# Edward-Sun/DIFUSCO

Measured on NVIDIA H100. Metric: TSP-500 graphs/sec, 50-step categorical denoise, higher is better.
Workload: dtype f32 (3-term bf16 split on wgmma, fp32 accumulate)

## Files before the change

### difusco_b200/_cabi.py

```python
import ctypes as C
import os

import numpy as np

HERE = os.path.dirname(os.path.abspath(__file__))
LIB_PATH = os.path.join(HERE, "libdifusco_b200.so")

DFB_OK, DFB_E_INVALID, DFB_E_CUDA, DFB_E_UNSUPPORTED, DFB_E_NOMEM = 0, -1, -2, -3, -4
CATEGORICAL, GAUSSIAN = 0, 1
EDGE_IMPL_TC, EDGE_IMPL_FP32, EDGE_IMPL_TC1 = 0, 1, 2
AGGREGATION = {"sum": 0, "mean": 1, "max": 2}
HEAD_FORWARD, HEAD_CATEGORICAL, HEAD_GAUSSIAN = 0, 1, 2

SYMBOLS = [
    "dfb_abi_version", "dfb_create", "dfb_destroy", "dfb_last_error", "dfb_set_aggregation",
    "dfb_set_edge_impl", "dfb_load_weights", "dfb_prepare_graph", "dfb_prepare_graph_instances", "dfb_set_points",
    "dfb_encoder_forward", "dfb_encoder_forward_timesteps", "dfb_denoise_step", "dfb_denoise", "dfb_denoise_record", "dfb_denoise_instances",
    "dfb_denoise_host",
    "dfb_launch_count", "dfb_profile_begin", "dfb_profile_end", "dfb_debug_edge_gemm", "dfb_debug_gnn_layer",
    "dfb_debug_gnn_layer_timesteps", "dfb_debug_head", "dfb_debug_entry", "dfb_debug_loop_captures",
    "dfb_debug_phase_cycles", "dfb_debug_watchdog", "dfb_knn_graph", "dfb_set_graph_capture",
    "dfb_set_phase_timing", "dfb_tsp_merge_sparse", "dfb_tsp_merge_order", "dfb_two_opt", "dfb_two_opt_instances",
    "dfb_write_heatmap_txt",
]

_lib = None


def lib():
  global _lib
  if _lib is not None:
    return _lib
  if not os.path.exists(LIB_PATH):
    raise RuntimeError(
        f"{LIB_PATH} not found: build it with `python -m difusco_b200.build` "
        "(difusco_b200 has no fallback path; the CUDA library is the product)")
  L = C.CDLL(LIB_PATH)
  vp, i32, i64, u64, f32 = C.c_void_p, C.c_int, C.c_int64, C.c_uint64, C.c_float
  L.dfb_abi_version.restype = i32
  L.dfb_create.argtypes = [C.POINTER(vp), i32]
  L.dfb_destroy.argtypes = [vp]
  L.dfb_last_error.argtypes = [vp]
  L.dfb_last_error.restype = C.c_char_p
  L.dfb_set_aggregation.argtypes = [vp, i32]
  L.dfb_set_edge_impl.argtypes = [vp, i32]
  L.dfb_load_weights.argtypes = [vp, i32, i32, i32, i32, i32, C.POINTER(C.c_char_p), C.POINTER(vp),
                                 C.POINTER(i64)]
  L.dfb_prepare_graph.argtypes = [vp, vp, i64, i64, i32, vp]
  L.dfb_prepare_graph_instances.argtypes = [vp, vp, i64, i64, i32, C.POINTER(i64), vp]
  L.dfb_set_points.argtypes = [vp, vp, vp]
  L.dfb_encoder_forward.argtypes = [vp, vp, f32, vp, vp]
  L.dfb_encoder_forward_timesteps.argtypes = [vp, vp, i32, C.POINTER(f32), vp, vp, vp]
  L.dfb_denoise_step.argtypes = [vp, i32, vp, f32, C.POINTER(f32), i32, vp, u64, i32, vp, vp, vp, vp]
  L.dfb_denoise.argtypes = [vp, i32, vp, i32, C.POINTER(C.c_int32), C.POINTER(f32),
                            C.POINTER(C.c_int32), vp, u64, vp]
  L.dfb_denoise_record.argtypes = [vp, i32, vp, i32, C.POINTER(C.c_int32), C.POINTER(f32), C.POINTER(C.c_int32), vp,
                                   u64, i32, C.POINTER(C.c_int32), vp, vp, vp, vp]
  L.dfb_denoise_instances.argtypes = [vp, i32, vp, i32, C.POINTER(C.c_int32), C.POINTER(f32), C.POINTER(C.c_int32),
                                      vp, i32, i32, C.POINTER(C.c_int32), vp, vp, vp, vp]
  L.dfb_denoise_host.argtypes = [vp, i32, vp, vp, i64, i64, i32, vp, i32, C.POINTER(C.c_int32),
                                 C.POINTER(f32), C.POINTER(C.c_int32), u64, vp, vp]
  L.dfb_launch_count.argtypes = [vp]
  L.dfb_launch_count.restype = i64
  L.dfb_debug_loop_captures.argtypes = [vp]
  L.dfb_debug_loop_captures.restype = i64
  L.dfb_profile_begin.argtypes = [vp]
  L.dfb_profile_end.argtypes = [vp, C.POINTER(C.c_double), C.POINTER(i64)]
  L.dfb_debug_edge_gemm.argtypes = [vp, i32, vp, vp, vp]
  L.dfb_debug_gnn_layer.argtypes = [vp, i32, f32, vp, vp, vp]
  L.dfb_debug_gnn_layer_timesteps.argtypes = [vp, i32, i32, C.POINTER(f32), vp, vp, vp, vp]
  L.dfb_debug_head.argtypes = [vp, i32, vp, C.POINTER(f32), i32, vp, u64, i32, vp, vp, vp, vp, vp, vp, vp]
  L.dfb_debug_entry.argtypes = [vp, i32, vp, f32, vp, vp, vp, vp, vp, vp]
  L.dfb_debug_phase_cycles.argtypes = [vp, C.POINTER(C.c_uint64)]
  L.dfb_debug_watchdog.argtypes = [vp, C.POINTER(C.c_int)]
  L.dfb_set_graph_capture.argtypes = [vp, i32]
  L.dfb_set_phase_timing.argtypes = [vp, i32]
  L.dfb_knn_graph.argtypes = [vp, vp, i64, i32, i64, vp, vp]
  L.dfb_tsp_merge_sparse.argtypes = [vp, i64, vp, vp, i64, i32, vp, C.POINTER(i64)]
  L.dfb_tsp_merge_order.argtypes = [i64, vp, i64, vp, C.POINTER(i64)]
  L.dfb_two_opt.argtypes = [vp, vp, i64, vp, i64, i64, C.POINTER(i64), vp]
  L.dfb_two_opt_instances.argtypes = [vp, vp, vp, i64, vp, vp, i64, vp, vp]
  L.dfb_write_heatmap_txt.argtypes = [C.c_char_p, i64, vp]
  for name in SYMBOLS:
    fn = getattr(L, name)
    if fn.restype is C.c_int and name not in ("dfb_abi_version",):
      fn.restype = i32
  _lib = L
  return L


class DfbError(RuntimeError):
  pass


def _raise(code, msg):
  msg = msg.decode() if isinstance(msg, bytes) else msg
  if code == DFB_E_INVALID:
    raise ValueError(msg)
  if code == DFB_E_UNSUPPORTED:
    raise NotImplementedError(msg)
  if code == DFB_E_NOMEM:
    raise MemoryError(msg)
  raise DfbError(msg)


MERGE_COMPLETE, MERGE_INCOMPLETE, MERGE_AMBIGUOUS = 0, 1, 2

# ... 212 lines not shown
                                         its.ctypes.data, stream))
    out, e = [], 0
    for p, t in zip(points_list, tours_list):
      b, n1 = np.shape(t)
      out.append(tours[e:e + b * n1].reshape(b, n1))
      e += b * n1
    return out, [int(x) for x in its]

  def knn_graph(self, points_ptr, num_nodes, k, node_offset, edge_index_ptr, stream=0):
    self._ck(lib().dfb_knn_graph(self._h, points_ptr, int(num_nodes), int(k), int(node_offset), edge_index_ptr, stream))

  def launch_count(self):
    return int(lib().dfb_launch_count(self._h))

  def loop_captures(self):
    return int(lib().dfb_debug_loop_captures(self._h))

  def profile_begin(self):
    self._ck(lib().dfb_profile_begin(self._h))

  def profile_end(self):
    ms, n = C.c_double(0), C.c_int64(0)
    self._ck(lib().dfb_profile_end(self._h, C.byref(ms), C.byref(n)))
    return ms.value, n.value

  def set_graph_capture(self, enabled):
    self._ck(lib().dfb_set_graph_capture(self._h, int(bool(enabled))))

  def debug_watchdog(self):
    out = (C.c_int * 4)()
    lib().dfb_debug_watchdog(self._h, out)
    return [int(x) for x in out]

  def set_phase_timing(self, enabled):
    self._ck(lib().dfb_set_phase_timing(self._h, int(bool(enabled))))

  def debug_phase_cycles(self):
    out = (C.c_uint64 * 32)()
    self._ck(lib().dfb_debug_phase_cycles(self._h, out))
    return [int(x) for x in out]

  def debug_edge_gemm(self, layer, e_in_ptr, acc_out_ptr, stream=0):
    self._ck(lib().dfb_debug_edge_gemm(self._h, layer, e_in_ptr, acc_out_ptr, stream))

  def debug_gnn_layer(self, layer, t, h_ptr, e_ptr, stream=0):
    self._ck(lib().dfb_debug_gnn_layer(self._h, int(layer), float(t), h_ptr, e_ptr, stream))

  def debug_gnn_layer_timesteps(self, layer, t_values, t_index_ptr, h_ptr, e_ptr, stream=0):
    v = np.ascontiguousarray(t_values, dtype=np.float32).reshape(-1)
    self._ck(lib().dfb_debug_gnn_layer_timesteps(self._h, int(layer), v.size, v.ctypes.data_as(C.POINTER(C.c_float)),
                                                 t_index_ptr, h_ptr, e_ptr, stream))

  def debug_head(self, mode, z_ptr, consts=(0, 0, 0, 0), last=0, uniforms_ptr=None, seed=0, step_index=0,
                 instance_seeds_ptr=None, xt_in_ptr=None, xt_out_ptr=None, p_out_ptr=None, net_out_ptr=None,
                 stats_out_ptr=None, stream=0):
    c = (C.c_float * 4)(*[float(x) for x in consts])
    self._ck(lib().dfb_debug_head(self._h, int(mode), z_ptr, c, int(last), uniforms_ptr,
                                  int(seed) & 0xFFFFFFFFFFFFFFFF, int(step_index), instance_seeds_ptr, xt_in_ptr,
                                  xt_out_ptr, p_out_ptr, net_out_ptr, stats_out_ptr, stream))

  def debug_entry(self, diffusion, xt_ptr, t, h0_out_ptr=None, e0_out_ptr=None, tvec_out_ptr=None, h_out_ptr=None,
                  e_out_ptr=None, stream=0):
    self._ck(lib().dfb_debug_entry(self._h, int(diffusion), xt_ptr, float(t), h0_out_ptr, e0_out_ptr, tvec_out_ptr,
                                   h_out_ptr, e_out_ptr, stream))
```

### difusco_b200/csrc/dfb_api.cu

```cuda
#include <cuda_runtime.h>
#include <math.h>
#include <stdio.h>
#include <stdlib.h>
#include <string.h>

#include <map>
#include <string>
#include <vector>

#include "../../include/difusco_b200.h"
#include "common.cuh"
#include "edge_layer_fp32.cuh"
#include "edge_layer_tc.cuh"
#include "kernels_small.cuh"
#include "knn.cuh"
#include "tsp_decode.cuh"

using namespace dfb;

static std::string g_create_error;

struct DevBuf {
  void* p = nullptr;
  size_t cap = 0;
// ... 1232 lines not shown
  ctx->h_tvals[slot][0] = t;
  ctx->h_steps[slot][0] = StepParams{};
  r = stage_commit(ctx, slot, 1, st);
  if (r) return r;
  const float* xt_lut;
  int e_zero;
  r = run_entry(ctx, mode, xt, &xt_lut, &e_zero, st);
  if (r) return r;
  const size_t V = ctx->g.V, E = ctx->g.E, row = H * sizeof(float);
  if (h0_out) CK(ctx, cudaMemcpyAsync(h0_out, ctx->h.p, V * row, cudaMemcpyDeviceToDevice, st));
  if (e0_out && xt_lut) {
    k_lut_expand<<<(ctx->g.E + 3) / 4, 256, 0, st>>>(xt_lut, ctx->g.perm, ctx->lut, e0_out, ctx->g.E);
    CKL(ctx);
  } else if (e0_out && !e_zero) {
    CK(ctx, cudaMemcpyAsync(e0_out, ctx->e.p, E * row, cudaMemcpyDeviceToDevice, st));
  }
  if (tvec_out) CK(ctx, cudaMemcpyAsync(tvec_out, ctx->tvec.p, ctx->L * row, cudaMemcpyDeviceToDevice, st));
  r = run_forward_layer(ctx, 0, (const float*)ctx->tvec.p, TimeRows{}, xt_lut, e_zero, st);
  if (r) return r;
  if (h_out) CK(ctx, cudaMemcpyAsync(h_out, ctx->h.p, V * row, cudaMemcpyDeviceToDevice, st));
  if (e_out) CK(ctx, cudaMemcpyAsync(e_out, ctx->e.p, E * row, cudaMemcpyDeviceToDevice, st));
  return DFB_OK;
}

extern "C" int dfb_debug_phase_cycles(dfb_ctx* ctx, unsigned long long* out) {
  if (!ctx || !out) return DFB_E_INVALID;
  CK(ctx, cudaSetDevice(ctx->device));
  CK(ctx, cudaDeviceSynchronize());
  CK(ctx, cudaMemcpy(out, ctx->tc.phase_cycles, 32 * sizeof(unsigned long long), cudaMemcpyDeviceToHost));
  CK(ctx, cudaMemset(ctx->tc.phase_cycles, 0, 32 * sizeof(unsigned long long)));
  return DFB_OK;
}

extern "C" int dfb_debug_watchdog(dfb_ctx* ctx, int* out) {
  if (!ctx || !out || !ctx->tc.error_host) return DFB_E_INVALID;
  for (int i = 0; i < 4; ++i) out[i] = ((volatile int*)ctx->tc.error_host)[i];
  return DFB_OK;
}

extern "C" int dfb_knn_graph(dfb_ctx* ctx, const double* points, int64_t num_nodes, int k, int64_t node_offset,
                             int64_t* edge_index, void* stream_) {
  if (!ctx) return DFB_E_INVALID;
  cudaStream_t st = (cudaStream_t)stream_;
  CK(ctx, cudaSetDevice(ctx->device));
  if (num_nodes < 1 || k < 1 || k > num_nodes) FAIL(ctx, DFB_E_INVALID, "bad kNN size N=%lld K=%d", (long long)num_nodes, k);
  if ((size_t)num_nodes * sizeof(double) > 200 * 1024) FAIL(ctx, DFB_E_UNSUPPORTED, "kNN graph: N=%lld exceeds the shared-memory brute-force limit (25600)", (long long)num_nodes);
  const size_t smem = (size_t)num_nodes * sizeof(double) + (size_t)(num_nodes + 31) / 32 * sizeof(unsigned);
  if (!is_device_ptr(edge_index)) FAIL(ctx, DFB_E_INVALID, "edge_index must be a device pointer");
  const double* dp = points;
  if (!is_device_ptr(points)) {
    for (int64_t i = 0; i < 2 * num_nodes; ++i)
      if (!std::isfinite(points[i])) FAIL(ctx, DFB_E_INVALID, "kNN graph: non-finite coordinate of node %lld", (long long)(i / 2));
    ENS_NOLOOP(ctx, ctx->d_points, (size_t)num_nodes * 2 * sizeof(double));
    CK(ctx, cudaMemcpyAsync(ctx->d_points.p, points, (size_t)num_nodes * 2 * sizeof(double), cudaMemcpyHostToDevice, st));
    dp = (const double*)ctx->d_points.p;
  }
  CK(ctx, cudaFuncSetAttribute(k_knn_bruteforce, cudaFuncAttributeMaxDynamicSharedMemorySize, (int)smem));
  k_knn_bruteforce<<<(int)num_nodes, 256, smem, st>>>(dp, (int)num_nodes, k, (long long*)edge_index, (long long)node_offset);
  CKL(ctx);
  return DFB_OK;
}

extern "C" int dfb_tsp_merge_sparse(const double* points, int64_t n, const float* heat, const int64_t* edge_index, int64_t E,
                                    int mode, int64_t* tour, int64_t* merge_iterations) {
  if (!points || !heat || !edge_index || !tour || !merge_iterations || n < 3 || n > 0x7fffffff / 2 || E < 0 || (mode != 0 && mode != 1))
    return DFB_E_INVALID;
// ... 146 lines not shown
```

### difusco_b200/csrc/edge_layer_tc.cuh

```cuda
#pragma once
#include <cuda.h>
#include <cuda_bf16.h>
#include <cuda_runtime.h>

#include <stdlib.h>

#include <string>

#include "common.cuh"
#include "edge_layer_fp32.cuh"

namespace dfb {

constexpr int WG_ROWS = 64;
constexpr int TC_KBLK = 64;
constexpr int TC_KCH = 32;
constexpr int TC_B_BYTES = 256 * TC_KCH * 2;
static_assert(TC_KCH * 2 == 64, "weight chunk rows are one 64-byte swizzle row (tensor map, wgmma_desc_sw64)");
constexpr int TC_A_CHUNK = WG_ROWS * 128;
constexpr int TC_A_BYTES = 8 * TC_A_CHUNK;
constexpr int CONV_BATCH = 16;

constexpr int W_LO_ROWS = H;
constexpr int W_MAT_ROWS = 2 * W_LO_ROWS;
// ... 56 lines not shown
  asm volatile("mbarrier.arrive.shared::cta.b64 _, [%0];" ::"r"(smem_u32(bar)) : "memory");
}
__device__ __forceinline__ void mbar_arrive_expect_tx(uint64_t* bar, uint32_t bytes) {
  asm volatile("mbarrier.arrive.expect_tx.shared::cta.b64 _, [%0], %1;" ::"r"(smem_u32(bar)), "r"(bytes) : "memory");
}
__device__ __forceinline__ void mbar_wait(uint64_t* bar, uint32_t parity, int* error_flag, int code) {
  const uint32_t addr = smem_u32(bar);
  uint32_t ok = 0;
#pragma unroll 1
  for (uint32_t spin = 0;; ++spin) {
    asm volatile(
        "{\n .reg .pred p;\n mbarrier.try_wait.parity.shared::cta.b64 p, [%1], %2, %3;\n selp.u32 %0, 1, 0, p;\n}"
        : "=r"(ok)
        : "r"(addr), "r"(parity), "r"(20000u)
        : "memory");
    if (ok) return;
    if (spin > 400000u) {
      if (error_flag) {
        error_flag[1] = (int)blockIdx.x;
        error_flag[2] = (int)parity;
        error_flag[3] = (int)threadIdx.x;
        atomicExch(error_flag, code);
      }
      __threadfence_system();
      __trap();
    }
  }
}
__device__ __forceinline__ void tma_load_2d(uint32_t dst, const CUtensorMap* map, uint64_t* bar, int c0, int c1) {
  asm volatile(
      "cp.async.bulk.tensor.2d.shared::cluster.global.mbarrier::complete_tx::bytes [%0], [%1, {%3, %4}], [%2];"
      ::"r"(dst), "l"(reinterpret_cast<uint64_t>(map)), "r"(smem_u32(bar)), "r"(c0), "r"(c1)
      : "memory");
}
__device__ __forceinline__ void fence_proxy_async() { asm volatile("fence.proxy.async.shared::cta;" ::: "memory"); }
__device__ __forceinline__ void cp_async16(void* dst, const void* src) {
  asm volatile("cp.async.cg.shared.global [%0], [%1], 16;" ::"r"(smem_u32(dst)), "l"(src) : "memory");
}
__device__ __forceinline__ void cp_async_commit() { asm volatile("cp.async.commit_group;" ::: "memory"); }
__device__ __forceinline__ void cp_async_wait_all() { asm volatile("cp.async.wait_group 0;" ::: "memory"); }

__device__ __forceinline__ uint64_t wgmma_desc_sw128(uint32_t smem_addr) {
  return (uint64_t)((smem_addr >> 4) & 0x3fffu) | (1ull << 16) | (64ull << 32) | (1ull << 62);
}
__device__ __forceinline__ uint64_t wgmma_desc_sw64(uint32_t smem_addr) {
  return (uint64_t)((smem_addr >> 4) & 0x3fffu) | (1ull << 16) | (32ull << 32) | (2ull << 62);
}
__device__ __forceinline__ void wgmma_fence() { asm volatile("wgmma.fence.sync.aligned;" ::: "memory"); }
__device__ __forceinline__ void wgmma_commit() { asm volatile("wgmma.commit_group.sync.aligned;" ::: "memory"); }
template <int N>
__device__ __forceinline__ void wgmma_wait() { asm volatile("wgmma.wait_group.sync.aligned %0;" ::"n"(N) : "memory"); }
__device__ __forceinline__ void acc_fence(float (&d)[128]) {
#pragma unroll
  for (int i = 0; i < 128; ++i) asm volatile("" : "+f"(d[i])::"memory");
}
__device__ __forceinline__ void wgmma_bf16(float (&d)[128], uint64_t da, uint64_t db, uint32_t scale_d) {
  asm volatile(
      "{\n .reg .pred p;\n setp.ne.b32 p, %130, 0;\n"
      "wgmma.mma_async.sync.aligned.m64n256k16.f32.bf16.bf16 "
      "{%0, %1, %2, %3, %4, %5, %6, %7, %8, %9, %10, %11, %12, %13, %14, %15, "
      "%16, %17, %18, %19, %20, %21, %22, %23, %24, %25, %26, %27, %28, %29, %30, %31, "
      "%32, %33, %34, %35, %36, %37, %38, %39, %40, %41, %42, %43, %44, %45, %46, %47, "
      "%48, %49, %50, %51, %52, %53, %54, %55, %56, %57, %58, %59, %60, %61, %62, %63, "
      "%64, %65, %66, %67, %68, %69, %70, %71, %72, %73, %74, %75, %76, %77, %78, %79, "
      "%80, %81, %82, %83, %84, %85, %86, %87, %88, %89, %90, %91, %92, %93, %94, %95, "
      "%96, %97, %98, %99, %100, %101, %102, %103, %104, %105, %106, %107, %108, %109, %110, %111, "
// ... 45 lines not shown
  return (uint32_t)((r >> 3) * 1024 + (r & 7) * 128 + ((j ^ (r & 7)) << 4));
}
__device__ __forceinline__ int msg_col(int j, int r) { return 64 * (j >> 3) + ((8 * (j & 7)) ^ (8 * (r & 7))); }
__device__ __forceinline__ float quad_sum(float v) {
  v += __shfl_xor_sync(0xffffffffu, v, 1);
  return v + __shfl_xor_sync(0xffffffffu, v, 2);
}
__device__ __forceinline__ void swap_row_halves(float (&d)[128]) {
#pragma unroll
  for (int j = 0; j < 32; ++j) {
    const float x0 = d[4 * j], x1 = d[4 * j + 1];
    d[4 * j] = d[4 * j + 2];
    d[4 * j + 1] = d[4 * j + 3];
    d[4 * j + 2] = x0;
    d[4 * j + 3] = x1;
  }
}

enum {
  PH_TILES = 0,
  PH_TOTAL,
  PH_CONVERT,
  PH_G1_WAIT,
  PH_G1_MMA,
  PH_E1,
  PH_REDUCE,
  PH_LN,
  PH_G2_WAIT,
  PH_G2_MMA,
  PH_E4,
  PH_COUNT
};

template <int NWG, bool LIN, bool TIMED = false, bool TROWS = false>
__device__ __forceinline__ void edge_layer_wg_body(const CUtensorMap& wmap, const TcParams& P) {
  using Cfg = TcCfg<NWG>;
  constexpr int NSTAGE = Cfg::NSTAGE;
  extern __shared__ unsigned char smem_raw[];
  unsigned char* smem = smem_raw + ((1024u - (smem_u32(smem_raw) & 1023u)) & 1023u);
  float* prm = reinterpret_cast<float*>(smem + Cfg::OFF_PRM);
  int* s_row = reinterpret_cast<int*>(smem + Cfg::OFF_ROW);
  const float** s_src = reinterpret_cast<const float**>(smem + Cfg::OFF_SRC);
  const float** s_tau = reinterpret_cast<const float**>(smem + Cfg::OFF_TAU);
  uint64_t* full = reinterpret_cast<uint64_t*>(smem + Cfg::OFF_BAR);
  uint64_t* empty = full + NSTAGE;

  const int warp = threadIdx.x >> 5, lane = threadIdx.x & 31;
  constexpr bool lin = LIN;
  const int loads_per_tile = (P.write_e ? 2 : 1) * NWG * 4 * NSTAGE;

  if (threadIdx.x == 0) {
    for (int s = 0; s < NSTAGE; ++s) {
      mbar_init(&full[s], 1);
      mbar_init(&empty[s], 4);
    }
    asm volatile("fence.mbarrier_init.release.cluster;" ::: "memory");
    fence_proxy_async();
  }
  for (int i = threadIdx.x; i < H; i += Cfg::THREADS) {
    prm[i] = P.lp.ln_e_g[i];
    prm[H + i] = P.lp.ln_e_b[i];
    prm[2 * H + i] = P.tvec ? P.tvec[i] : 0.0f;
    prm[3 * H + i] = P.lp.ln_o_g[i];
    prm[4 * H + i] = P.lp.ln_o_b[i];
    prm[5 * H + i] = P.lp.b_O[i];
  }
  __syncthreads();
  const uint32_t smem_base = smem_u32(smem);

  if (warp >= 4 * NWG) {
    if constexpr (NWG == 2) asm volatile("setmaxnreg.dec.sync.aligned.u32 40;" ::: "memory");
    if (warp == 4 * NWG && lane == 0) {
      uint32_t u = 0;
      for (int tile = blockIdx.x; tile < P.n_tiles; tile += gridDim.x) {
        for (int i = 0; i < loads_per_tile; ++i, ++u) {
          const int s = u % NSTAGE;
          mbar_wait(&empty[s], ((u / NSTAGE) & 1) ^ 1, P.error_flag, 1);
          mbar_arrive_expect_tx(&full[s], TC_B_BYTES);
          const int row = (lin ? P.lin_w_row + (P.lin_nb == 4 ? (tile & 3) : 0) * W_MAT_ROWS
                               : P.w_row_base + (i >= 4 * NSTAGE * NWG ? w_row_O(0) - w_row_C(0) : 0)) +
                          (s >= NSTAGE / 2 ? W_LO_ROWS : 0);
          const int k = ((i / NSTAGE) & 3) * TC_KBLK + (s % (NSTAGE / 2)) * TC_KCH;
          tma_load_2d(smem_base + Cfg::OFF_B + s * TC_B_BYTES, &wmap, &full[s], k, row);
        }
      }
    }
    return;
  }

  if constexpr (NWG == 2) asm volatile("setmaxnreg.inc.sync.aligned.u32 232;" ::: "memory");
  const int wg = warp >> 2, wi = warp & 3, tid = threadIdx.x & 127;
  const int t4 = lane & 3;
  const int lr0 = wi * 16 + (lane >> 2);
  unsigned char* a_reg = smem + wg * TC_A_BYTES;
  const uint32_t a_base = smem_base + wg * TC_A_BYTES;
  float* msg = reinterpret_cast<float*>(a_reg);
  int* w_row = s_row + wg * WG_ROWS;
  const float** w_src = s_src + wg * WG_ROWS;
  const float** w_tau = s_tau + wg * WG_ROWS;
  auto wg_bar = [&] { asm volatile("bar.sync %0, 128;" ::"r"(1 + wg) : "memory"); };
  const int n_rows = lin ? P.lin_rows : P.g.E;
  float acc[128];

  auto turn_wait = [&] {
    if constexpr (NWG == 2) asm volatile("bar.sync %0, 256;" ::"r"(3 + wg) : "memory");
  };
  auto turn_pass = [&] {
    if constexpr (NWG == 2) asm volatile("bar.arrive %0, 256;" ::"r"(4 - wg) : "memory");
  };
  if (wg == 1) turn_pass();

  uint32_t t_mark = 0, t_start = 0;
  if constexpr (TIMED) t_start = t_mark = (uint32_t)clock();
  auto record = [&](int slot, uint32_t v) {
    if constexpr (TIMED) {
      if (tid == 0) atomicAdd(P.phase_cycles + slot, (unsigned long long)v);
    }
  };
  auto mark = [&](int slot) {
    if constexpr (TIMED) {
      const uint32_t now = (uint32_t)clock();
      record(slot, now - t_mark);
      t_mark = now;
    }
  };

  auto gemm = [&](int wait_slot, int mma_slot) {
    uint32_t waited = 0;
    turn_wait();
    if constexpr (TIMED) t_mark = (uint32_t)clock();
    acc_fence(acc);
    wgmma_fence();
#pragma unroll 1
    for (int kc = 0; kc < 4; ++kc) {
      const uint32_t ahi = a_base + kc * 2 * TC_A_CHUNK, alo = ahi + TC_A_CHUNK;
#pragma unroll
      for (int s = 0; s < NSTAGE; ++s) {
        uint32_t w0 = 0;
        if constexpr (TIMED) w0 = (uint32_t)clock();
        mbar_wait(&full[s], kc & 1, P.error_flag, 2);
        if constexpr (TIMED) waited += (uint32_t)clock() - w0;
        const uint32_t b = smem_base + Cfg::OFF_B + s * TC_B_BYTES;
        const bool b_hi = s < NSTAGE / 2;
#pragma unroll
        for (int k = 0; k < TC_KCH / 16; ++k) {
          const int ks = (s % (NSTAGE / 2)) * (TC_KCH / 16) + k;
          const uint64_t db = wgmma_desc_sw64(b + k * 32);
          wgmma_bf16(acc, wgmma_desc_sw128(ahi + ks * 32), db, (b_hi && ks == 0) ? (uint32_t)(kc != 0) : 1u);
          if (b_hi) wgmma_bf16(acc, wgmma_desc_sw128(alo + ks * 32), db, 1u);
        }
        wgmma_commit();
        wgmma_wait<1>();
        __syncwarp();
        if (lane == 0 && (s > 0 || kc > 0)) mbar_arrive(&empty[(s + NSTAGE - 1) % NSTAGE]);
      }
    }
    wgmma_wait<0>();
    acc_fence(acc);
    __syncwarp();
    if (lane == 0) mbar_arrive(&empty[NSTAGE - 1]);
    turn_pass();
    if constexpr (TIMED) {
      const uint32_t now = (uint32_t)clock();
      record(wait_slot, waited);
      record(mma_slot, now - t_mark - waited);
      t_mark = now;
    }
  };

  auto stage_rows = [&](auto row_src) {
#pragma unroll 1
    for (int i = 0; i < 16; ++i) {
      const int r = wi * 16 + i;
      const float* src = row_src(i) + 4 * lane;
      float* dst = msg + r * H + ((4 * lane) ^ (8 * (r & 7)));
      cp_async16(dst, src);
      cp_async16(dst + 128, src + 128);
    }
    cp_async_commit();
  };

  for (int tile = blockIdx.x; tile < P.n_tiles; tile += gridDim.x) {
    record(PH_TILES, 1);
    const int row_tile = (lin && P.lin_nb == 4) ? (tile >> 2) : tile;
    const int s_base = row_tile * Cfg::TILE + wg * WG_ROWS;
    if (tid < WG_ROWS) {
      const int s = s_base + tid;
      const float* src = P.zero_row;
      int rw = -1;
      if (s < n_rows && lin) {
        src = P.lin_in + (size_t)s * H;
      } else if (s < n_rows) {
        rw = P.g.row[s];
        if (P.e_zero) src = P.zero_row;
        else if (P.xt_lut) src = P.lut + ((P.xt_lut[P.g.perm ? P.g.perm[s] : s] != 0.0f) ? H : 0);
        else src = P.e + (size_t)s * H;
      }
      w_row[tid] = rw;
      w_src[tid] = src;
      if constexpr (TROWS) w_tau[tid] = s < n_rows ? time_row(P.tvec, P.trows, P.g.perm ? P.g.perm[s] : s) : P.zero_row;
    }
    wg_bar();

#pragma unroll 1
    for (int it0 = 0; it0 < 32; it0 += CONV_BATCH) {
      float4 x[CONV_BATCH];
#pragma unroll
      for (int q = 0; q < CONV_BATCH; ++q) {
        const int item = (it0 + q) * 128 + tid;
        x[q] = __ldcg(reinterpret_cast<const float4*>(w_src[item >> 6]) + (item & 63));
      }
#pragma unroll
      for (int q = 0; q < CONV_BATCH; ++q) {
        const int item = (it0 + q) * 128 + tid;
        const int rr = item >> 6, k4 = item & 63;
        uint2 hi, lo;
        split4(x[q], hi, lo);
        const uint32_t off = (k4 >> 4) * 2 * TC_A_CHUNK + sw128_off(rr, (k4 & 15) >> 1) + (k4 & 1) * 8;
        *reinterpret_cast<uint2*>(a_reg + off) = hi;
        *reinterpret_cast<uint2*>(a_reg + off + TC_A_CHUNK) = lo;
      }
    }
    fence_proxy_async();
    wg_bar();
    mark(PH_CONVERT);
    gemm(PH_G1_WAIT, PH_G1_MMA);

    const int sa = s_base + lr0, sb = sa + 8;
    const bool va = sa < n_rows, vb = sb < n_rows;
    if (lin || P.debug_acc) {
      const int nb = (lin && P.lin_nb == 4) ? (tile & 3) : 0;
      const int ostride = lin ? P.lin_nb * H : H;
      float* out = lin ? P.lin_out + nb * H : P.debug_acc;
#pragma unroll
      for (int h = 0; h < 2; ++h) {
        const int s = h ? sb : sa;
        if (!(h ? vb : va)) continue;
#pragma unroll
        for (int j = 0; j < 32; ++j) {
          const int c = 8 * j + 2 * t4;
          float2 o = make_float2(acc[4 * j + 2 * h], acc[4 * j + 2 * h + 1]);
          if (lin) {
            const float2 bb = __ldg(reinterpret_cast<const float2*>(P.lin_bias + nb * H + c));
            o.x += bb.x;
            o.y += bb.y;
          }
          __stcg(reinterpret_cast<float2*>(out + (size_t)s * ostride + c), o);
        }
      }
      continue;
    }

    const int s_lane = s_base + wi * 16 + (lane & 15);
    const int col_lane = s_lane < n_rows ? P.g.col[s_lane] : 0;
    stage_rows([&](int i) { return P.uvab + (size_t)__shfl_sync(0xffffffffu, col_lane, i) * 4 * H + H; });
#pragma unroll 1
    for (int h = 0; h < 2; ++h) {
      const bool v = h ? vb : va;
      const float* ap = P.uvab + (size_t)__shfl_sync(0xffffffffu, col_lane, (lane >> 2) + 8 * h) * 4 * H + 2 * H;
      const float* bp = P.uvab + (size_t)(v ? P.g.row[h ? sb : sa] : 0) * 4 * H + 3 * H;
#pragma unroll
      for (int j = 0; j < 32; ++j) {
        const int c = 8 * j + 2 * t4;
        const float2 ah = __ldg(reinterpret_cast<const float2*>(ap + c));
        const float2 bh = __ldg(reinterpret_cast<const float2*>(bp + c));
        acc[4 * j] = (acc[4 * j] + ah.x) + bh.x;
        acc[4 * j + 1] = (acc[4 * j + 1] + ah.y) + bh.y;
      }
      if (h == 0) {
        cp_async_wait_all();
        __syncwarp();
      }
      float* m = msg + (lr0 + 8 * h) * H + 2 * t4;
#pragma unroll
      for (int j = 0; j < 32; ++j) {
        float2* mp = reinterpret_cast<float2*>(m + msg_col(j, lr0));
        const float2 vh = *mp;
        *mp = make_float2(sigmoid_mufu(acc[4 * j]) * vh.x, sigmoid_mufu(acc[4 * j + 1]) * vh.y);
      }
      swap_row_halves(acc);
    }
    wg_bar();
    mark(PH_E1);
    const bool amax = P.agg_mode == AGG_MAX;
    const float run0 = amax ? -INFINITY : 0.0f;
#pragma unroll 1
    for (int g2 = 0; g2 < WG_ROWS / GROUP; ++g2) {
      const int grp = (s_base >> 5) + g2;
      if (grp >= P.g.n_groups) break;
      const int first_node = P.g.grp_first[grp];
      const size_t pair_base = (size_t)P.g.grp_pair[grp];
      const int node = w_row[g2 * GROUP + lane];
      const int nxt = __shfl_down_sync(0xffffffffu, node, 1);
      const uint32_t ends = __ballot_sync(0xffffffffu, node >= 0 && (lane == GROUP - 1 || nxt != node));
#pragma unroll 1
      for (int cc = 0; cc < 2; ++cc) {
        const int c = tid + 128 * cc;
        float run = run0;
#pragma unroll 8
        for (int r = 0; r < GROUP; ++r) {
          const int lr = g2 * GROUP + r;
          const float m = msg[lr * H + (c ^ (8 * (lr & 7)))];
          run = amax ? fmaxf(run, m) : run + m;
          if ((ends >> r) & 1u) {
            P.partials[(pair_base + (size_t)(w_row[lr] - first_node)) * H + c] = run;
            run = run0;
          }
        }
      }
    }
    wg_bar();
    mark(PH_REDUCE);
    if (!P.write_e) continue;

#pragma unroll 1
    for (int h = 0; h < 2; ++h) {
      float sum = 0.f;
#pragma unroll
      for (int j = 0; j < 32; ++j) sum += acc[4 * j] + acc[4 * j + 1];
      float mean = quad_sum(sum) * (1.0f / H);
      float q = 0.f;
#pragma unroll
      for (int j = 0; j < 32; ++j) {
        const float d0 = acc[4 * j] - mean, d1 = acc[4 * j + 1] - mean;
        q = fmaf(d0, d0, fmaf(d1, d1, q));
      }
      float rstd = rsqrtf(quad_sum(q) * (1.0f / H) + LN_EPS);
      sum = 0.f;
      const float* tau = nullptr;
      if constexpr (TROWS) tau = w_tau[lr0 + 8 * h];
#pragma unroll
      for (int j = 0; j < 32; ++j) {
        const int c = 8 * j + 2 * t4;
        const float2 g = *reinterpret_cast<const float2*>(prm + c);
        const float2 b = *reinterpret_cast<const float2*>(prm + H + c);
        float2 t;
        if constexpr (TROWS) t = __ldg(reinterpret_cast<const float2*>(tau + c));
        else t = *reinterpret_cast<const float2*>(prm + 2 * H + c);
        const float y0 = fmaxf(fmaf((acc[4 * j] - mean) * rstd, g.x, b.x), 0.0f) + t.x;
        const float y1 = fmaxf(fmaf((acc[4 * j + 1] - mean) * rstd, g.y, b.y), 0.0f) + t.y;
        acc[4 * j] = y0;
        acc[4 * j + 1] = y1;
        sum += y0 + y1;
      }
      mean = quad_sum(sum) * (1.0f / H);
      q = 0.f;
// ... 16 lines not shown
        const uint32_t off = (j >> 3) * 2 * TC_A_CHUNK + sw128_off(r, j & 7) + 4 * t4;
        *reinterpret_cast<uint32_t*>(a_reg + off) = hi;
        *reinterpret_cast<uint32_t*>(a_reg + off + TC_A_CHUNK) = lo;
      }
      swap_row_halves(acc);
    }
    const float* e_src = w_src[wi * 16 + (lane & 15)];
    fence_proxy_async();
    wg_bar();
    mark(PH_LN);
    gemm(PH_G2_WAIT, PH_G2_MMA);

    stage_rows([&](int i) {
      return reinterpret_cast<const float*>(__shfl_sync(0xffffffffu, reinterpret_cast<unsigned long long>(e_src), i));
    });
    cp_async_wait_all();
    __syncwarp();
#pragma unroll
    for (int h = 0; h < 2; ++h) {
      if (!(h ? vb : va)) continue;
      const int r = lr0 + 8 * h;
      const float* er = msg + r * H + 2 * t4;
      float* dst = P.e + (size_t)(h ? sb : sa) * H;
#pragma unroll
      for (int j = 0; j < 32; ++j) {
        const int c = 8 * j + 2 * t4;
        const float2 ein = *reinterpret_cast<const float2*>(er + msg_col(j, r));
        const float2 bo = *reinterpret_cast<const float2*>(prm + 5 * H + c);
        __stcg(reinterpret_cast<float2*>(dst + c),
               make_float2((ein.x + acc[4 * j + 2 * h]) + bo.x, (ein.y + acc[4 * j + 2 * h + 1]) + bo.y));
      }
    }
    mark(PH_E4);
  }
  if constexpr (TIMED) record(PH_TOTAL, (uint32_t)clock() - t_start);
}

__global__ void __launch_bounds__(TcCfg<2>::THREADS, 1)
k_edge_layer_wg2(const __grid_constant__ CUtensorMap wmap, const TcParams P) {
  edge_layer_wg_body<2, false>(wmap, P);
}
__global__ void __launch_bounds__(TcCfg<2>::THREADS, 1)
k_edge_layer_wg2_timed(const __grid_constant__ CUtensorMap wmap, const TcParams P) {
  edge_layer_wg_body<2, false, true>(wmap, P);
}
__global__ void __launch_bounds__(TcCfg<1>::THREADS, 1)
k_edge_layer_wg1(const __grid_constant__ CUtensorMap wmap, const TcParams P) {
  edge_layer_wg_body<1, false>(wmap, P);
}
__global__ void __launch_bounds__(TcCfg<2>::THREADS, 1)
k_edge_layer_wg2_trows(const __grid_constant__ CUtensorMap wmap, const TcParams P) {
  edge_layer_wg_body<2, false, false, true>(wmap, P);
}
__global__ void __launch_bounds__(TcCfg<1>::THREADS, 1)
k_edge_layer_wg1_trows(const __grid_constant__ CUtensorMap wmap, const TcParams P) {
  edge_layer_wg_body<1, false, false, true>(wmap, P);
}
__global__ void __launch_bounds__(TcCfg<2>::THREADS, 1)
k_linear_wg2(const __grid_constant__ CUtensorMap wmap, const TcParams P) {
  edge_layer_wg_body<2, true>(wmap, P);
}

struct TcState {
  std::string err;
  int num_sms = 0;
  CUtensorMap wmap;
  bool bound = false;
  float* zero_row = nullptr;
  int* error_flag = nullptr;
  int* error_host = nullptr;
  unsigned long long* phase_cycles = nullptr;

  TcState() = default;
  TcState(const TcState&) = delete;
  TcState& operator=(const TcState&) = delete;
  ~TcState() {
    if (zero_row) cudaFree(zero_row);
    if (error_host) cudaFreeHost(error_host);
    if (phase_cycles) cudaFree(phase_cycles);
  }
};

typedef CUresult (*PFN_encodeTiled)(CUtensorMap*, CUtensorMapDataType, cuuint32_t, void*, const cuuint64_t*,
                                    const cuuint64_t*, const cuuint32_t*, const cuuint32_t*, CUtensorMapInterleave,
                                    CUtensorMapSwizzle, CUtensorMapL2promotion, CUtensorMapFloatOOBfill);

inline int tc_init(TcState* st, int num_sms) {
  st->num_sms = num_sms;
  cudaError_t e = cudaFuncSetAttribute(k_edge_layer_wg2, cudaFuncAttributeMaxDynamicSharedMemorySize, TcCfg<2>::SMEM_ALLOC);
  if (e == cudaSuccess)
    e = cudaFuncSetAttribute(k_edge_layer_wg2_timed, cudaFuncAttributeMaxDynamicSharedMemorySize, TcCfg<2>::SMEM_ALLOC);
  if (e == cudaSuccess)
    e = cudaFuncSetAttribute(k_edge_layer_wg1, cudaFuncAttributeMaxDynamicSharedMemorySize, TcCfg<1>::SMEM_ALLOC);
  if (e == cudaSuccess)
    e = cudaFuncSetAttribute(k_edge_layer_wg2_trows, cudaFuncAttributeMaxDynamicSharedMemorySize, TcCfg<2>::SMEM_ALLOC_TROWS);
  if (e == cudaSuccess)
    e = cudaFuncSetAttribute(k_edge_layer_wg1_trows, cudaFuncAttributeMaxDynamicSharedMemorySize, TcCfg<1>::SMEM_ALLOC_TROWS);
  if (e == cudaSuccess)
    e = cudaFuncSetAttribute(k_linear_wg2, cudaFuncAttributeMaxDynamicSharedMemorySize, TcCfg<2>::SMEM_ALLOC);
  if (e != cudaSuccess) {
    st->err = std::string("cudaFuncSetAttribute: ") + cudaGetErrorString(e);
    return -2;
  }
  if ((e = cudaMalloc(&st->zero_row, H * sizeof(float))) != cudaSuccess ||
      (e = cudaMemset(st->zero_row, 0, H * sizeof(float))) != cudaSuccess ||
      (e = cudaMalloc(&st->phase_cycles, 32 * sizeof(unsigned long long))) != cudaSuccess ||
      (e = cudaMemset(st->phase_cycles, 0, 32 * sizeof(unsigned long long))) != cudaSuccess ||
      (e = cudaHostAlloc(&st->error_host, 4 * sizeof(int), cudaHostAllocMapped)) != cudaSuccess ||
      (e = cudaHostGetDevicePointer((void**)&st->error_flag, st->error_host, 0)) != cudaSuccess) {
    st->err = std::string("tc_init alloc: ") + cudaGetErrorString(e);
    return -2;
  }
  return 0;
}

inline int tc_bind_weights(TcState* st, const uint16_t* arena, int L) {
  void* fn = nullptr;
  cudaDriverEntryPointQueryResult qres;
  cudaError_t e = cudaGetDriverEntryPoint("cuTensorMapEncodeTiled", &fn, cudaEnableDefault, &qres);
  if (e != cudaSuccess || !fn || qres != cudaDriverEntryPointSuccess) {
    st->err = "cuTensorMapEncodeTiled entry point not available";
    cudaGetLastError();
    return -2;
  }
  cuuint64_t gdim[2] = {(cuuint64_t)H, (cuuint64_t)w_arena_rows(L)};
  cuuint64_t gstride[1] = {(cuuint64_t)H * sizeof(uint16_t)};
  cuuint32_t box[2] = {(cuuint32_t)TC_KCH, 256u};
  cuuint32_t estr[2] = {1u, 1u};
  CUresult r = ((PFN_encodeTiled)fn)(&st->wmap, CU_TENSOR_MAP_DATA_TYPE_BFLOAT16, 2, (void*)arena, gdim,
                                     gstride, box, estr, CU_TENSOR_MAP_INTERLEAVE_NONE, CU_TENSOR_MAP_SWIZZLE_64B,
                                     CU_TENSOR_MAP_L2_PROMOTION_L2_256B, CU_TENSOR_MAP_FLOAT_OOB_FILL_NONE);
  if (r != CUDA_SUCCESS) {
    st->err = "cuTensorMapEncodeTiled failed with CUresult " + std::to_string((int)r);
    return -2;
  }
  st->bound = true;
  return 0;
}

template <int NWG>
inline int tc_launch(TcState* st, void (*kernel)(CUtensorMap, TcParams), TcParams& P, int rows, int nb,
                     cudaStream_t stream, int smem = TcCfg<NWG>::SMEM_ALLOC) {
  if (!st->bound) {
    st->err = "weights not bound";
    return -1;
  }
  P.zero_row = st->zero_row; P.error_flag = st->error_flag; P.phase_cycles = st->phase_cycles;
  P.n_tiles = nb * ((rows + TcCfg<NWG>::TILE - 1) / TcCfg<NWG>::TILE);
  const int grid = P.n_tiles < st->num_sms ? P.n_tiles : st->num_sms;
  kernel<<<grid, TcCfg<NWG>::THREADS, smem, stream>>>(st->wmap, P);
  const cudaError_t err = cudaGetLastError();
  if (err == cudaSuccess) return 0;
  st->err = std::string("launch: ") + cudaGetErrorString(err);
  return -2;
}

inline int tc_launch_edge_layer(TcState* st, int l, float* e, const float* uvab, float* partials, const GraphDev& g,
                                const LayerParams& lp, const float* tvec, const TimeRows& trows, int write_e,
                                int e_zero, const float* xt_lut, const float* lut, int agg_mode, int nwg, bool timed,
                                float* debug_acc, cudaStream_t stream) {
  TcParams P{};
  P.e = e; P.uvab = uvab; P.partials = partials; P.g = g; P.lp = lp; P.tvec = tvec;
  P.xt_lut = xt_lut; P.lut = lut; P.debug_acc = debug_acc;
  P.write_e = debug_acc ? 0 : write_e;
  P.e_zero = e_zero; P.agg_mode = agg_mode;
  P.w_row_base = w_row_C(l);
  if (trows.index && tvec && !debug_acc) {
    P.trows = trows;
    if (nwg == 1) return tc_launch<1>(st, k_edge_layer_wg1_trows, P, g.E, 1, stream, TcCfg<1>::SMEM_ALLOC_TROWS);
    return tc_launch<2>(st, k_edge_layer_wg2_trows, P, g.E, 1, stream, TcCfg<2>::SMEM_ALLOC_TROWS);
  }
  if (nwg == 1) return tc_launch<1>(st, k_edge_layer_wg1, P, g.E, 1, stream);
  return tc_launch<2>(st, timed && !debug_acc ? k_edge_layer_wg2_timed : k_edge_layer_wg2, P, g.E, 1, stream);
}

inline int tc_launch_linear(TcState* st, const float* in, float* out, const float* bias, int rows, int nb, int w_row,
                            cudaStream_t stream) {
  TcParams P{};
  P.lin_in = in; P.lin_out = out; P.lin_bias = bias; P.lin_rows = rows; P.lin_nb = nb; P.lin_w_row = w_row;
  P.lp.ln_e_g = P.lp.ln_e_b = P.lp.ln_o_g = P.lp.ln_o_b = P.lp.b_O = st->zero_row;
  return tc_launch<2>(st, k_linear_wg2, P, rows, nb, stream);
}

}
```

### include/difusco_b200.h

```cpp
#ifndef DIFUSCO_B200_H_
#define DIFUSCO_B200_H_

#include <stdint.h>

#ifdef __cplusplus
extern "C" {
#endif

#define DFB_ABI_VERSION 2

enum {
  DFB_OK = 0,
  DFB_E_INVALID = -1,
  DFB_E_CUDA = -2,
  DFB_E_UNSUPPORTED = -3,
  DFB_E_NOMEM = -4
};

enum { DFB_TASK_TSP = 0, DFB_TASK_MIS = 1 };
enum { DFB_DIFFUSION_CATEGORICAL = 0, DFB_DIFFUSION_GAUSSIAN = 1 };
enum { DFB_EDGE_IMPL_TC = 0, DFB_EDGE_IMPL_FP32 = 1, DFB_EDGE_IMPL_TC1 = 2 };
enum { DFB_HEAD_FORWARD = 0, DFB_HEAD_CATEGORICAL = 1, DFB_HEAD_GAUSSIAN = 2 };

typedef struct dfb_ctx dfb_ctx;
// ... 64 lines not shown
int dfb_two_opt_instances(dfb_ctx* ctx, const double* points, const int64_t* node_ptr, int64_t n_instances,
                          const int64_t* tour_ptr, int64_t* tours, int64_t max_iterations, int64_t* iterations_out,
                          void* stream);

int dfb_write_heatmap_txt(const char* path, int64_t n, const double* matrix);

int64_t dfb_launch_count(const dfb_ctx* ctx);

int dfb_profile_begin(dfb_ctx* ctx);
int dfb_profile_end(dfb_ctx* ctx, double* edge_kernel_ms, int64_t* edge_kernel_launches);

int dfb_debug_edge_gemm(dfb_ctx* ctx, int layer, const float* e_in, float* acc_out, void* stream);

int dfb_debug_gnn_layer(dfb_ctx* ctx, int layer, float t, float* h, float* e, void* stream);

int dfb_debug_gnn_layer_timesteps(dfb_ctx* ctx, int layer, int n_t, const float* t_values, const int32_t* t_index,
                                  float* h, float* e, void* stream);

int dfb_debug_head(dfb_ctx* ctx, int mode, const float* z, const float* consts, int last, const float* uniforms,
                   uint64_t seed, int step_index, const uint64_t* instance_seeds, const float* xt_in, float* xt_out,
                   float* p_out, float* net_out, float* stats_out, void* stream);

int dfb_debug_entry(dfb_ctx* ctx, int diffusion_type, const float* xt, float t, float* h0_out, float* e0_out,
                    float* tvec_out, float* h_out, float* e_out, void* stream);

int64_t dfb_debug_loop_captures(const dfb_ctx* ctx);

int dfb_debug_phase_cycles(dfb_ctx* ctx, unsigned long long* out);

int dfb_set_phase_timing(dfb_ctx* ctx, int enabled);

int dfb_debug_watchdog(dfb_ctx* ctx, int* out);

#ifdef __cplusplus
}
#endif
#endif
```

Measured before the change: 23.49.

## Multicast edge-layer weight tiles across 2-CTA clusters via TMA

Launches the two-warpgroup edge GEMM kernels as 2-CTA clusters. Rank 0 issues TMA multicast loads of each weight stage to both CTAs, and consumers release stages on both CTAs' empty barriers, which roughly halves L2 weight traffic. Grid size is now bounded by the occupancy-derived maximum active clusters. Small grids fall back to a non-clustered solo kernel. The change adds cross-CTA synchronization, including a cluster barrier at the last tile, so a slow partner CTA can stall the other.

```diff
diff --git a/difusco_b200/_cabi.py b/difusco_b200/_cabi.py
--- a/difusco_b200/_cabi.py
+++ b/difusco_b200/_cabi.py
@@ -19,7 +19,7 @@
     "dfb_denoise_host",
     "dfb_launch_count", "dfb_profile_begin", "dfb_profile_end", "dfb_debug_edge_gemm", "dfb_debug_gnn_layer",
     "dfb_debug_gnn_layer_timesteps", "dfb_debug_head", "dfb_debug_entry", "dfb_debug_loop_captures",
-    "dfb_debug_phase_cycles", "dfb_debug_watchdog", "dfb_knn_graph", "dfb_set_graph_capture",
+    "dfb_debug_phase_cycles", "dfb_debug_watchdog", "dfb_debug_edge_clusters", "dfb_knn_graph", "dfb_set_graph_capture",
     "dfb_set_phase_timing", "dfb_tsp_merge_sparse", "dfb_tsp_merge_order", "dfb_two_opt", "dfb_two_opt_instances",
     "dfb_write_heatmap_txt",
 ]
@@ -73,6 +73,7 @@
   L.dfb_debug_entry.argtypes = [vp, i32, vp, f32, vp, vp, vp, vp, vp, vp]
   L.dfb_debug_phase_cycles.argtypes = [vp, C.POINTER(C.c_uint64)]
   L.dfb_debug_watchdog.argtypes = [vp, C.POINTER(C.c_int)]
+  L.dfb_debug_edge_clusters.argtypes = [vp, C.POINTER(C.c_int)]
   L.dfb_set_graph_capture.argtypes = [vp, i32]
   L.dfb_set_phase_timing.argtypes = [vp, i32]
   L.dfb_knn_graph.argtypes = [vp, vp, i64, i32, i64, vp, vp]
@@ -351,6 +352,11 @@
     lib().dfb_debug_watchdog(self._h, out)
     return [int(x) for x in out]
 
+  def debug_edge_clusters(self):
+    out = (C.c_int * 3)()
+    self._ck(lib().dfb_debug_edge_clusters(self._h, out))
+    return [int(x) for x in out]
+
   def set_phase_timing(self, enabled):
     self._ck(lib().dfb_set_phase_timing(self._h, int(bool(enabled))))
 
diff --git a/difusco_b200/csrc/dfb_api.cu b/difusco_b200/csrc/dfb_api.cu
--- a/difusco_b200/csrc/dfb_api.cu
+++ b/difusco_b200/csrc/dfb_api.cu
@@ -1288,6 +1288,14 @@
   return DFB_OK;
 }
 
+extern "C" int dfb_debug_edge_clusters(dfb_ctx* ctx, int* out) {
+  if (!ctx || !out) return DFB_E_INVALID;
+  out[0] = ctx->tc.clusters_wg2;
+  out[1] = ctx->tc.clusters_wg2_timed;
+  out[2] = ctx->tc.clusters_wg2_trows;
+  return DFB_OK;
+}
+
 extern "C" int dfb_debug_watchdog(dfb_ctx* ctx, int* out) {
   if (!ctx || !out || !ctx->tc.error_host) return DFB_E_INVALID;
   for (int i = 0; i < 4; ++i) out[i] = ((volatile int*)ctx->tc.error_host)[i];
diff --git a/difusco_b200/csrc/edge_layer_tc.cuh b/difusco_b200/csrc/edge_layer_tc.cuh
--- a/difusco_b200/csrc/edge_layer_tc.cuh
+++ b/difusco_b200/csrc/edge_layer_tc.cuh
@@ -112,6 +112,29 @@
       "cp.async.bulk.tensor.2d.shared::cluster.global.mbarrier::complete_tx::bytes [%0], [%1, {%3, %4}], [%2];"
       ::"r"(dst), "l"(reinterpret_cast<uint64_t>(map)), "r"(smem_u32(bar)), "r"(c0), "r"(c1)
       : "memory");
+}
+__device__ __forceinline__ void tma_load_2d_multicast(uint32_t dst, const CUtensorMap* map, uint64_t* bar, int c0, int c1,
+                                                      uint16_t mask) {
+  asm volatile(
+      "cp.async.bulk.tensor.2d.shared::cluster.global.mbarrier::complete_tx::bytes.multicast::cluster"
+      " [%0], [%1, {%3, %4}], [%2], %5;"
+      ::"r"(dst), "l"(reinterpret_cast<uint64_t>(map)), "r"(smem_u32(bar)), "r"(c0), "r"(c1), "h"(mask)
+      : "memory");
+}
+__device__ __forceinline__ uint32_t cluster_ctarank() {
+  uint32_t r;
+  asm volatile("mov.u32 %0, %%cluster_ctarank;" : "=r"(r));
+  return r;
+}
+__device__ __forceinline__ void mbar_arrive_cluster(uint64_t* bar, uint32_t rank) {
+  asm volatile(
+      "{\n .reg .b32 ra;\n mapa.shared::cluster.u32 ra, %0, %1;\n"
+      " mbarrier.arrive.shared::cluster.b64 _, [ra];\n}"
+      ::"r"(smem_u32(bar)), "r"(rank)
+      : "memory");
+}
+__device__ __forceinline__ void cluster_sync() {
+  asm volatile("barrier.cluster.arrive.release;\n barrier.cluster.wait.acquire;" ::: "memory");
 }
 __device__ __forceinline__ void fence_proxy_async() { asm volatile("fence.proxy.async.shared::cta;" ::: "memory"); }
 __device__ __forceinline__ void cp_async16(void* dst, const void* src) {
@@ -223,8 +246,9 @@
   PH_COUNT
 };
 
-template <int NWG, bool LIN, bool TIMED = false, bool TROWS = false>
+template <int NWG, bool LIN, bool TIMED = false, bool TROWS = false, int CLUSTER = 1>
 __device__ __forceinline__ void edge_layer_wg_body(const CUtensorMap& wmap, const TcParams& P) {
+  static_assert(CLUSTER == 1 || (CLUSTER == 2 && NWG == 2 && !LIN), "2-CTA clusters run the two-warpgroup edge kernels");
   using Cfg = TcCfg<NWG>;
   constexpr int NSTAGE = Cfg::NSTAGE;
   extern __shared__ unsigned char smem_raw[];
@@ -237,13 +261,14 @@
   uint64_t* empty = full + NSTAGE;
 
   const int warp = threadIdx.x >> 5, lane = threadIdx.x & 31;
+  const int rank = (int)(blockIdx.x % CLUSTER);
   constexpr bool lin = LIN;
   const int loads_per_tile = (P.write_e ? 2 : 1) * NWG * 4 * NSTAGE;
 
   if (threadIdx.x == 0) {
     for (int s = 0; s < NSTAGE; ++s) {
       mbar_init(&full[s], 1);
-      mbar_init(&empty[s], 4);
+      mbar_init(&empty[s], 4 * CLUSTER);
     }
     asm volatile("fence.mbarrier_init.release.cluster;" ::: "memory");
     fence_proxy_async();
@@ -256,26 +281,33 @@
     prm[4 * H + i] = P.lp.ln_o_b[i];
     prm[5 * H + i] = P.lp.b_O[i];
   }
-  __syncthreads();
+  if constexpr (CLUSTER > 1) cluster_sync();
+  else __syncthreads();
   const uint32_t smem_base = smem_u32(smem);
 
   if (warp >= 4 * NWG) {
     if constexpr (NWG == 2) asm volatile("setmaxnreg.dec.sync.aligned.u32 40;" ::: "memory");
     if (warp == 4 * NWG && lane == 0) {
       uint32_t u = 0;
-      for (int tile = blockIdx.x; tile < P.n_tiles; tile += gridDim.x) {
+      for (int tile0 = blockIdx.x - rank; tile0 < P.n_tiles; tile0 += gridDim.x) {
+        const int tile = tile0 + rank;
         for (int i = 0; i < loads_per_tile; ++i, ++u) {
           const int s = u % NSTAGE;
           mbar_wait(&empty[s], ((u / NSTAGE) & 1) ^ 1, P.error_flag, 1);
           mbar_arrive_expect_tx(&full[s], TC_B_BYTES);
+          if (CLUSTER > 1 && rank != 0) continue;
           const int row = (lin ? P.lin_w_row + (P.lin_nb == 4 ? (tile & 3) : 0) * W_MAT_ROWS
                                : P.w_row_base + (i >= 4 * NSTAGE * NWG ? w_row_O(0) - w_row_C(0) : 0)) +
                           (s >= NSTAGE / 2 ? W_LO_ROWS : 0);
           const int k = ((i / NSTAGE) & 3) * TC_KBLK + (s % (NSTAGE / 2)) * TC_KCH;
-          tma_load_2d(smem_base + Cfg::OFF_B + s * TC_B_BYTES, &wmap, &full[s], k, row);
+          if constexpr (CLUSTER > 1)
+            tma_load_2d_multicast(smem_base + Cfg::OFF_B + s * TC_B_BYTES, &wmap, &full[s], k, row, (1u << CLUSTER) - 1);
+          else
+            tma_load_2d(smem_base + Cfg::OFF_B + s * TC_B_BYTES, &wmap, &full[s], k, row);
         }
       }
     }
+    if constexpr (CLUSTER > 1) cluster_sync();
     return;
   }
 
@@ -316,6 +348,10 @@
     }
   };
 
+  auto release = [&](uint64_t* bar) {
+    mbar_arrive(bar);
+    if constexpr (CLUSTER > 1) mbar_arrive_cluster(bar, rank ^ 1);
+  };
   auto gemm = [&](int wait_slot, int mma_slot) {
     uint32_t waited = 0;
     turn_wait();
@@ -343,13 +379,13 @@
         wgmma_commit();
         wgmma_wait<1>();
         __syncwarp();
-        if (lane == 0 && (s > 0 || kc > 0)) mbar_arrive(&empty[(s + NSTAGE - 1) % NSTAGE]);
+        if (lane == 0 && (s > 0 || kc > 0)) release(&empty[(s + NSTAGE - 1) % NSTAGE]);
       }
     }
     wgmma_wait<0>();
     acc_fence(acc);
     __syncwarp();
-    if (lane == 0) mbar_arrive(&empty[NSTAGE - 1]);
+    if (lane == 0) release(&empty[NSTAGE - 1]);
     turn_pass();
     if constexpr (TIMED) {
       const uint32_t now = (uint32_t)clock();
@@ -371,8 +407,14 @@
     cp_async_commit();
   };
 
-  for (int tile = blockIdx.x; tile < P.n_tiles; tile += gridDim.x) {
-    record(PH_TILES, 1);
+  auto tile_done = [&](int tile0) {
+    if constexpr (CLUSTER > 1) {
+      if (tile0 + (int)gridDim.x >= P.n_tiles) cluster_sync();
+    }
+  };
+  for (int tile0 = blockIdx.x - rank; tile0 < P.n_tiles; tile0 += gridDim.x) {
+    const int tile = tile0 + rank;
+    if (tile < P.n_tiles) record(PH_TILES, 1);
     const int row_tile = (lin && P.lin_nb == 4) ? (tile >> 2) : tile;
     const int s_base = row_tile * Cfg::TILE + wg * WG_ROWS;
     if (tid < WG_ROWS) {
@@ -439,6 +481,7 @@
           __stcg(reinterpret_cast<float2*>(out + (size_t)s * ostride + c), o);
         }
       }
+      tile_done(tile0);
       continue;
     }
 
@@ -502,7 +545,10 @@
     }
     wg_bar();
     mark(PH_REDUCE);
-    if (!P.write_e) continue;
+    if (!P.write_e) {
+      tile_done(tile0);
+      continue;
+    }
 
 #pragma unroll 1
     for (int h = 0; h < 2; ++h) {
@@ -585,25 +631,30 @@
       }
     }
     mark(PH_E4);
+    tile_done(tile0);
   }
   if constexpr (TIMED) record(PH_TOTAL, (uint32_t)clock() - t_start);
 }
 
+__global__ void __cluster_dims__(2, 1, 1) __launch_bounds__(TcCfg<2>::THREADS, 1)
+k_edge_layer_wg2(const __grid_constant__ CUtensorMap wmap, const TcParams P) {
+  edge_layer_wg_body<2, false, false, false, 2>(wmap, P);
+}
+__global__ void __cluster_dims__(2, 1, 1) __launch_bounds__(TcCfg<2>::THREADS, 1)
+k_edge_layer_wg2_timed(const __grid_constant__ CUtensorMap wmap, const TcParams P) {
+  edge_layer_wg_body<2, false, true, false, 2>(wmap, P);
+}
 __global__ void __launch_bounds__(TcCfg<2>::THREADS, 1)
-k_edge_layer_wg2(const __grid_constant__ CUtensorMap wmap, const TcParams P) {
+k_edge_layer_wg2_solo(const __grid_constant__ CUtensorMap wmap, const TcParams P) {
   edge_layer_wg_body<2, false>(wmap, P);
-}
-__global__ void __launch_bounds__(TcCfg<2>::THREADS, 1)
-k_edge_layer_wg2_timed(const __grid_constant__ CUtensorMap wmap, const TcParams P) {
-  edge_layer_wg_body<2, false, true>(wmap, P);
 }
 __global__ void __launch_bounds__(TcCfg<1>::THREADS, 1)
 k_edge_layer_wg1(const __grid_constant__ CUtensorMap wmap, const TcParams P) {
   edge_layer_wg_body<1, false>(wmap, P);
 }
-__global__ void __launch_bounds__(TcCfg<2>::THREADS, 1)
+__global__ void __cluster_dims__(2, 1, 1) __launch_bounds__(TcCfg<2>::THREADS, 1)
 k_edge_layer_wg2_trows(const __grid_constant__ CUtensorMap wmap, const TcParams P) {
-  edge_layer_wg_body<2, false, false, true>(wmap, P);
+  edge_layer_wg_body<2, false, false, true, 2>(wmap, P);
 }
 __global__ void __launch_bounds__(TcCfg<1>::THREADS, 1)
 k_edge_layer_wg1_trows(const __grid_constant__ CUtensorMap wmap, const TcParams P) {
@@ -617,6 +668,7 @@
 struct TcState {
   std::string err;
   int num_sms = 0;
+  int clusters_wg2 = 0, clusters_wg2_timed = 0, clusters_wg2_trows = 0;
   CUtensorMap wmap;
   bool bound = false;
   float* zero_row = nullptr;
@@ -643,6 +695,8 @@
   cudaError_t e = cudaFuncSetAttribute(k_edge_layer_wg2, cudaFuncAttributeMaxDynamicSharedMemorySize, TcCfg<2>::SMEM_ALLOC);
   if (e == cudaSuccess)
     e = cudaFuncSetAttribute(k_edge_layer_wg2_timed, cudaFuncAttributeMaxDynamicSharedMemorySize, TcCfg<2>::SMEM_ALLOC);
+  if (e == cudaSuccess)
+    e = cudaFuncSetAttribute(k_edge_layer_wg2_solo, cudaFuncAttributeMaxDynamicSharedMemorySize, TcCfg<2>::SMEM_ALLOC);
   if (e == cudaSuccess)
     e = cudaFuncSetAttribute(k_edge_layer_wg1, cudaFuncAttributeMaxDynamicSharedMemorySize, TcCfg<1>::SMEM_ALLOC);
   if (e == cudaSuccess)
@@ -655,6 +709,21 @@
     st->err = std::string("cudaFuncSetAttribute: ") + cudaGetErrorString(e);
     return -2;
   }
+  auto max_clusters = [&](const void* kernel, int smem, int* out) {
+    cudaLaunchConfig_t cfg = {};
+    cfg.gridDim = dim3(2);
+    cfg.blockDim = dim3(TcCfg<2>::THREADS);
+    cfg.dynamicSmemBytes = smem;
+    cudaError_t r = cudaOccupancyMaxActiveClusters(out, kernel, &cfg);
+    return r == cudaSuccess && *out < 1 ? cudaErrorInvalidConfiguration : r;
+  };
+  if ((e = max_clusters((const void*)k_edge_layer_wg2, TcCfg<2>::SMEM_ALLOC, &st->clusters_wg2)) != cudaSuccess ||
+      (e = max_clusters((const void*)k_edge_layer_wg2_timed, TcCfg<2>::SMEM_ALLOC, &st->clusters_wg2_timed)) != cudaSuccess ||
+      (e = max_clusters((const void*)k_edge_layer_wg2_trows, TcCfg<2>::SMEM_ALLOC_TROWS, &st->clusters_wg2_trows)) !=
+          cudaSuccess) {
+    st->err = std::string("cudaOccupancyMaxActiveClusters: ") + cudaGetErrorString(e);
+    return -2;
+  }
   if ((e = cudaMalloc(&st->zero_row, H * sizeof(float))) != cudaSuccess ||
       (e = cudaMemset(st->zero_row, 0, H * sizeof(float))) != cudaSuccess ||
       (e = cudaMalloc(&st->phase_cycles, 32 * sizeof(unsigned long long))) != cudaSuccess ||
@@ -693,14 +762,16 @@
 
 template <int NWG>
 inline int tc_launch(TcState* st, void (*kernel)(CUtensorMap, TcParams), TcParams& P, int rows, int nb,
-                     cudaStream_t stream, int smem = TcCfg<NWG>::SMEM_ALLOC) {
+                     cudaStream_t stream, int smem = TcCfg<NWG>::SMEM_ALLOC, int max_clusters = 0) {
   if (!st->bound) {
     st->err = "weights not bound";
     return -1;
   }
   P.zero_row = st->zero_row; P.error_flag = st->error_flag; P.phase_cycles = st->phase_cycles;
   P.n_tiles = nb * ((rows + TcCfg<NWG>::TILE - 1) / TcCfg<NWG>::TILE);
-  const int grid = P.n_tiles < st->num_sms ? P.n_tiles : st->num_sms;
+  const int pairs = (P.n_tiles + 1) / 2;
+  const int grid = max_clusters > 0 ? 2 * (pairs < max_clusters ? pairs : max_clusters)
+                                    : (P.n_tiles < st->num_sms ? P.n_tiles : st->num_sms);
   kernel<<<grid, TcCfg<NWG>::THREADS, smem, stream>>>(st->wmap, P);
   const cudaError_t err = cudaGetLastError();
   if (err == cudaSuccess) return 0;
@@ -721,10 +792,15 @@
   if (trows.index && tvec && !debug_acc) {
     P.trows = trows;
     if (nwg == 1) return tc_launch<1>(st, k_edge_layer_wg1_trows, P, g.E, 1, stream, TcCfg<1>::SMEM_ALLOC_TROWS);
-    return tc_launch<2>(st, k_edge_layer_wg2_trows, P, g.E, 1, stream, TcCfg<2>::SMEM_ALLOC_TROWS);
+    return tc_launch<2>(st, k_edge_layer_wg2_trows, P, g.E, 1, stream, TcCfg<2>::SMEM_ALLOC_TROWS,
+                        st->clusters_wg2_trows);
   }
   if (nwg == 1) return tc_launch<1>(st, k_edge_layer_wg1, P, g.E, 1, stream);
-  return tc_launch<2>(st, timed && !debug_acc ? k_edge_layer_wg2_timed : k_edge_layer_wg2, P, g.E, 1, stream);
+  if (timed && !debug_acc)
+    return tc_launch<2>(st, k_edge_layer_wg2_timed, P, g.E, 1, stream, TcCfg<2>::SMEM_ALLOC, st->clusters_wg2_timed);
+  if ((g.E + TcCfg<2>::TILE - 1) / TcCfg<2>::TILE <= st->num_sms)
+    return tc_launch<2>(st, k_edge_layer_wg2_solo, P, g.E, 1, stream);
+  return tc_launch<2>(st, k_edge_layer_wg2, P, g.E, 1, stream, TcCfg<2>::SMEM_ALLOC, st->clusters_wg2);
 }
 
 inline int tc_launch_linear(TcState* st, const float* in, float* out, const float* bias, int rows, int nb, int w_row,
diff --git a/include/difusco_b200.h b/include/difusco_b200.h
--- a/include/difusco_b200.h
+++ b/include/difusco_b200.h
@@ -120,6 +120,8 @@
 
 int dfb_debug_watchdog(dfb_ctx* ctx, int* out);
 
+int dfb_debug_edge_clusters(dfb_ctx* ctx, int* out);
+
 #ifdef __cplusplus
 }
 #endif
```

New measurement: 23.80, median of 6. +1.3%, better.
